# chongkuiqi/S2ANet

Measured on AMD Instinct MI355X. Metric: 1024x1024 DOTA chips/sec (R-50-FPN S2ANet inference), higher is better.
Workload: dtype f16; 1 GPU; BASELINE configs[2]: full R-50-FPN S2ANet inference, batch 8 of 1024x1024 synthetic uint8 chips per GPU; 3 independent batches in flight on 3 HIP streams; global_batch=8, num_classes=15, weights=seeded random init of the reference architecture; odm_cls bias calibrated, nms_candidate_cap=160000, nms_candidates_dropped=0, distinct_input_batches=3, fam_cls_branch=True, hip_graph=False, batches_in_flight=3, parallelism=dp1 (one process per GPU)

## Files before the change

include/s2anet_hip.h:

```cpp
#ifndef S2ANET_HIP_H_
#define S2ANET_HIP_H_

#include <stddef.h>
#include <stdint.h>

#ifdef __cplusplus
extern "C" {
#endif

#define S2A_OK 0
#define S2A_EINVAL (-1)
#define S2A_EWORKSPACE (-2)
#define S2A_EHIP (-3)
#define S2A_ENOTIMPL (-4)

#define S2A_DTYPE_F32 0
#define S2A_DTYPE_F16 1
#define S2A_DTYPE_F64 2

#define S2A_LAYOUT_NCHW 0
#define S2A_LAYOUT_NHWC 1

typedef void* s2a_stream_t;

// ... 237 lines not shown
                                                int64_t out_channels);
int s2a_deform_conv_backward(int dtype, const void* input, const void* offset, const void* grad_output, const void* weight,
                             float* grad_input_f32, void* grad_offset, float* grad_weight_f32, float scale, int64_t batch,
                             int64_t channels, int64_t height, int64_t width, int64_t out_channels, void* workspace,
                             size_t workspace_bytes, s2a_stream_t stream);
int s2a_deform_conv_backward_typed(int dtype, const void* input, const void* offset, const void* grad_output,
                                   const void* weight, void* grad_input, void* grad_offset, float* grad_weight_f32,
                                   float scale, int64_t batch, int64_t channels, int64_t height, int64_t width,
                                   int64_t out_channels, void* workspace, size_t workspace_bytes, s2a_stream_t stream);

int s2a_conv3x3_tail1x1_f16(const void* x, const void* weight_frag, const void* bias, const void* tail_weight_frag,
                            const void* tail_bias, const void* residual, void* out, const void* chain_weight_frag,
                            const void* chain_bias, void* chain_out, int64_t chain_channels, int64_t batch, int64_t channels,
                            int64_t mid_channels, int64_t out_channels, int64_t height, int64_t width,
                            s2a_stream_t stream);

int s2a_conv1x1_chain_f16(const void* x, const void* weight_frag, const void* bias, const void* residual, void* out,
                          const void* chain_weight_frag, const void* chain_bias, void* chain_out, int64_t chain_channels,
                          int64_t batch, int64_t channels, int64_t out_channels, int64_t height, int64_t width,
                          s2a_stream_t stream);

int s2a_conv1x1_add_up2_f16(const void* x, const void* weight_frag, const void* bias, const void* coarse,
                            void* out, int64_t batch, int64_t channels, int64_t height, int64_t width,
                            int64_t out_channels, s2a_stream_t stream);

int64_t s2a_pyramid_pixels(const s2a_pyramid* pyr, int64_t batch);
int s2a_conv3x3_pyramid_f16(const void* x, const void* weight_frag, const void* bias, const void* residual,
                            void* out, int64_t batch, int64_t channels, int64_t out_channels, int relu,
                            const s2a_pyramid* pyr, s2a_stream_t stream);
int s2a_conv3x3_head_pyramid_f16(const void* x, const void* weight_frag, const void* bias, void* out,
// ... 115 lines not shown
```

s2anet_amd/_lib.py:

```python
import ctypes
import os
import subprocess

import torch

_HERE = os.path.dirname(os.path.abspath(__file__))
LIB_PATH = os.environ.get("S2A_LIB_PATH") or os.path.join(_HERE, "libs2anet_hip.so")

OK, EINVAL, EWORKSPACE, EHIP, ENOTIMPL = 0, -1, -2, -3, -4
DTYPE_F32, DTYPE_F16, DTYPE_F64 = 0, 1, 2
LAYOUT_NCHW, LAYOUT_NHWC = 0, 1

c_i64, c_int, c_f32, c_sz, c_vp = (ctypes.c_int64, ctypes.c_int, ctypes.c_float, ctypes.c_size_t,
                                   ctypes.c_void_p)


class DcnParams(ctypes.Structure):
    _fields_ = [("batch", c_i64), ("channels", c_i64), ("height", c_i64), ("width", c_i64),
                ("out_channels", c_i64),
                ("kW", c_int), ("kH", c_int), ("dW", c_int), ("dH", c_int), ("padW", c_int),
                ("padH", c_int), ("dilationW", c_int), ("dilationH", c_int), ("group", c_int),
                ("deformable_group", c_int), ("dtype", c_int), ("offset_dtype", c_int),
                ("layout", c_int), ("relu", c_int)]

# ... 129 lines not shown
    "s2a_deform_conv_backward_typed": (c_int, [c_int, c_vp, c_vp, c_vp, c_vp, c_vp, c_vp, c_vp, c_f32, c_i64, c_i64, c_i64, c_i64,
                                               c_i64, c_vp, c_sz, c_vp]),
    "s2a_deform_conv_backward_input_f32_workspace_bytes": (c_sz, [c_i64, c_i64, c_i64, c_i64, c_i64]),
    "s2a_deform_conv_backward_weight_f32_workspace_bytes": (c_sz, [c_i64, c_i64, c_i64, c_i64, c_i64]),
    "s2a_deform_conv_backward_weight_f32": (c_int, [c_vp, c_vp, c_vp, c_vp, c_f32, c_i64, c_i64, c_i64, c_i64, c_i64,
                                                    c_vp, c_sz, c_vp]),
    "s2a_deform_conv_backward_input_f32": (c_int, [c_vp, c_vp, c_vp, c_vp, c_vp, c_vp, c_i64, c_i64, c_i64, c_i64, c_i64,
                                                   c_vp, c_sz, c_vp]),
    "s2a_deform_conv_backward_weight_f16": (c_int, [c_vp, c_vp, c_vp, c_vp, c_i64, c_i64, c_i64, c_i64, c_i64, c_vp, c_sz, c_vp]),
    "s2a_deform_conv_backward_input_f16": (c_int, [c_vp, c_vp, c_vp, c_vp, c_vp, c_vp, c_i64, c_i64, c_i64, c_i64, c_i64,
                                           c_vp, c_sz, c_vp]),
    "s2a_deformable_im2col": (c_int, [c_vp, c_vp, c_vp, ctypes.POINTER(DcnParams), c_vp]),
    "s2a_deformable_col2im": (c_int, [c_vp, c_vp, c_vp, ctypes.POINTER(DcnParams), c_vp]),
    "s2a_deformable_col2im_coord": (c_int, [c_vp, c_vp, c_vp, c_vp, ctypes.POINTER(DcnParams), c_vp]),
    "s2a_conv3x3_tail1x1_f16": (c_int, [c_vp] * 10 + [c_i64] * 7 + [c_vp]),
    "s2a_conv1x1_chain_f16": (c_int, [c_vp] * 8 + [c_i64] * 6 + [c_vp]),
    "s2a_conv1x1_add_up2_f16": (c_int, [c_vp, c_vp, c_vp, c_vp, c_vp, c_i64, c_i64, c_i64, c_i64, c_i64, c_vp]),
    "s2a_pyramid_pixels": (c_i64, [ctypes.POINTER(Pyramid), c_i64]),
    "s2a_conv3x3_pyramid_f16": (c_int, [c_vp, c_vp, c_vp, c_vp, c_vp, c_i64, c_i64, c_i64, c_int,
                                        ctypes.POINTER(Pyramid), c_vp]),
    "s2a_conv3x3_head_pyramid_f16": (c_int, [c_vp, c_vp, c_vp, c_vp, c_vp, c_vp, c_vp, c_i64, c_i64, c_i64, c_int,
                                             ctypes.POINTER(Pyramid), c_vp]),
    "s2a_conv3x3_narrow_pyramid_f16": (c_int, [c_vp, c_vp, c_vp, c_vp, c_i64, c_i64, c_i64, c_int, ctypes.POINTER(Pyramid), c_vp]),
    "s2a_orconv_pool_pyramid_f16": (c_int, [c_vp, c_vp, c_vp, c_vp, c_vp, c_i64, c_i64, c_i64, ctypes.POINTER(Pyramid), c_vp]),
    "s2a_conv_wino_packed_elems": (c_i64, [c_i64, c_i64]),
    "s2a_conv_wino_pack_weight_f16": (c_int, [c_vp, c_i64, c_i64, c_vp, c_vp]),
    "s2a_conv3x3_wino_pyramid_f16": (c_int, [c_vp, c_vp, c_vp, c_vp, c_vp, c_i64, c_i64, c_i64, c_int,
                                             ctypes.POINTER(Pyramid), c_vp]),
    "s2a_quantize_e4m3": (c_int, [c_vp, c_vp, c_i64, c_i64, c_f32, c_vp]),
    "s2a_conv_pack_weight_fp8": (c_int, [c_vp, c_i64, c_i64, c_vp, c_vp]),
# ... 102 lines not shown
```

s2anet_amd/csrc/conv_ops.hip:

```cpp
#include <hip/hip_fp16.h>
#include <hip/hip_runtime.h>

#include <algorithm>
#include <cstdlib>
#include <type_traits>

#include "common.hpp"
#include "mfma_common.hpp"

namespace s2a {
namespace {

__global__ void k_pack_weight_frag(const _Float16* __restrict__ w, int O, int C, _Float16* __restrict__ wp,
                                   int taps = 9) {
  int64_t e = (int64_t)blockIdx.x * blockDim.x + threadIdx.x;
  int64_t total = (int64_t)O * C * taps;
  if (e >= total) return;
  const int G = O / 64;
  int j = (int)(e & 7);
  int lane = (int)((e >> 3) & 63);
  int kk = (int)((e >> 9) & 3);
  int mt = (int)((e >> 11) & 1);
  int64_t r = e >> 12;
  int g = (int)(r % G);
// ... 8 lines not shown

struct ConvExtra {
  _Float16* pool_out;
  const _Float16* head_w;
  const _Float16* head_b;
  _Float16* head_out;
  int store_main;
  const _Float16* tail_w;
  const _Float16* tail_b;
  const _Float16* tail_res;
  _Float16* tail_out;
  const _Float16* chain_w;
  const _Float16* chain_b;
  _Float16* chain_out;
  int chain_O;
};

template <int TAPS, int OG, int PH = 1, int SD = 1, bool TAIL = false, int HT = 0>
struct ConvCfg {
  static constexpr int kTH = (SD == 2 || HT) ? 4 : 8 * PH;
  static constexpr int kPos = (SD == 2 || HT) ? 64 : 128 * PH;
  static constexpr int kWaves = 4 * PH;
  static constexpr int kPW = SD == 2 ? 33 : kCPW;
  static constexpr int kNT = (kPos / 32) * OG / 4 / PH;
  static constexpr int kPix = TAPS == 9 ? ((kTH - 1) * SD + 3) * kPW : kPos;
  static constexpr int kDma = (kPix * 9 + 63) / 64;
  static constexpr int kPatchBytes = kDma * 1024;
  static constexpr int kOutRowB = OG * 128 + 16;
  static constexpr bool kWLds = PH == 2 && TAPS == 9;
  static constexpr int kWBuf = OG * 8192;
  static constexpr int kLoop0 = 2 * kPatchBytes + (kWLds ? 2 * kWBuf : 0);
  static constexpr int kLoop = (kWLds && OG == 1 && kPatchBytes + 9 * 8192 > kLoop0) ? kPatchBytes + 9 * 8192 : kLoop0;
  static constexpr int kLds0 = (kLoop > kPos * kOutRowB) ? kLoop : kPos * kOutRowB;
  static constexpr int kTailRowB = 528;
  static constexpr int kLds = (TAIL && kPos * kTailRowB > kLds0) ? kPos * kTailRowB : kLds0;
  static constexpr int kBiasBytes = TAIL ? 1024 : 512;
  static constexpr int kJ = (kDma + kWaves - 1) / kWaves;
};

template <int TAPS, int OG, int PH = 1, int SD = 1, bool TAIL = false, int HT = 0>
__global__ __launch_bounds__(256 * PH, PH == 1 ? 2 : 1) void k_conv_f16(const _Float16* __restrict__ x_,
                                                     const _Float16* __restrict__ wfrag,
                                                     const _Float16* __restrict__ bias,
                                                     const _Float16* __restrict__ residual_,
                                                     _Float16* __restrict__ out_, int64_t Ntot_, int C,
                                                     int H_, int W_, int Ho_, int Wo_, int cstride, int O,
                                                     int relu, unsigned x_bytes_, LevelTab lt, int res_up,
                                                     ConvExtra ex) {
  _Float16* pool_out_ = ex.pool_out;
  using T = _Float16;
  using V = f16x8;
  using Cfg = ConvCfg<TAPS, OG, PH, SD, TAIL, HT>;
  constexpr int NT = Cfg::kNT;
  static_assert(NT >= 1, "unsupported tile / group combination");
  static_assert(!HT || (TAPS == 9 && PH == 1 && SD == 1 && !TAIL), "half tiles: plain 3x3 / stride 1");
  static_assert(!TAIL || (TAPS == 9 && OG == 1 && SD == 1), "the fused 1x1 tail follows a 64-map 3x3/s1");
  constexpr int WPG = 4 / OG;
  constexpr int kThreads_ = 256 * PH;
  extern __shared__ __attribute__((aligned(16))) char smem[];
  const int tid = threadIdx.x, lane = tid & 63, wave = tid >> 6;
  const int wave4 = wave & 3, blk = wave >> 2;
  int64_t tile = xcd_remap(blockIdx.x, gridDim.x);
  const T* x = x_;
  const T* residual = residual_;
  T* out = out_;
  int64_t Ntot = Ntot_;
  int H = H_, W = W_, Ho = Ho_, Wo = Wo_;
  unsigned x_bytes = x_bytes_;
  if (TAPS == 9 && lt.n > 1) {
    int t0 = 0, p0 = 0;
#pragma unroll
// ... 136 lines not shown
      return;
    }
#pragma unroll
    for (int kk = 0; kk < 4; kk++) {
      V pf[NT];
#pragma unroll
      for (int b = 0; b < NT; b++) pf[b] = *reinterpret_cast<const V*>(P + fbase[b] + toff + kk * 32);
#pragma unroll
      for (int a = 0; a < 2; a++)
#pragma unroll
        for (int b = 0; b < NT; b++)
          acc[a][b] = __builtin_amdgcn_mfma_f32_32x32x16_f16(wv[a][kk], pf[b], acc[a][b], 0, 0, 0);
    }
  };

  constexpr bool kEarlyRes = TAIL && Cfg::kWLds;
  constexpr int NI2 = TAIL ? Cfg::kPos * 32 / kThreads_ : 1;
  unsigned off2[NI2];
  V r2[NI2];
  auto tail_res_issue = [&]() {
    const __amdgpu_buffer_rsrc_t rr = __builtin_amdgcn_make_buffer_rsrc(
        const_cast<T*>(ex.tail_res ? ex.tail_res : ex.tail_out), 0, (int)((uint64_t)Ntot * 256 * 2), 0x00020000);
#pragma unroll
    for (int i = 0; i < NI2; i++) {
      const int idx = tid + kThreads_ * i, pos = idx >> 5, col = idx & 31;
      const int64_t gp = tile_pos(tile, pos, Cfg::kTH, Ho, Wo, HWo, Ntot);
      off2[i] = gp >= 0 ? (unsigned)((gp * 256 + col * 8) * 2) : 0x80000000u;
      r2[i] = __builtin_bit_cast(V, __builtin_amdgcn_raw_buffer_load_b128(rr, (int)(ex.tail_res ? off2[i] : 0x80000000u), 0, 0));
    }
  };
  const int nstage = TAPS * CC, last = nstage - 1;
  if constexpr (Cfg::kWLds) {
    char* wb = smem + 2 * Cfg::kPatchBytes;
    const __amdgpu_buffer_rsrc_t rw = __builtin_amdgcn_make_buffer_rsrc(
// ... 154 lines not shown
          const int och = grp * 64 + 32 * a + 8 * rq + 4 * (lane >> 5);
          const h4e bq = *reinterpret_cast<const h4e*>(s_bias + och);
#pragma unroll
          for (int b = 0; b < NT; b++) {
            int pos = 128 * blk + 32 * (sub * NT + b) + lp;
            *reinterpret_cast<h4e*>(s_out + pos * Cfg::kOutRowB + och * 2) =
                quad(acc[a][b][rq * 4], acc[a][b][rq * 4 + 1], acc[a][b][rq * 4 + 2], acc[a][b][rq * 4 + 3], bq);
          }
        }
    }
  };
  if (wave_active) {
    if (relu && !residual) stage_tile(std::true_type{}); else stage_tile(std::false_type{});
  }
  __syncthreads();
  if constexpr (TAIL) {
    f32x4 acc3s[4][8];
    {
#pragma unroll
      for (int a = 0; a < 4; a++)
#pragma unroll
        for (int b = 0; b < 8; b++)
#pragma unroll
          for (int r = 0; r < 4; r++) acc3s[a][b][r] = 0.f;
      const char* brow = s_out + (128 * blk + pix16) * Cfg::kOutRowB + (kg16 & 1) * 64 + (kg16 >> 1) * 16;
#pragma unroll
      for (int ks = 0; ks < 2; ks++)
#pragma unroll
        for (int bh = 0; bh < 8; bh += 4) {
          V pf[4];
#pragma unroll
          for (int b = 0; b < 4; b++) pf[b] = *reinterpret_cast<const V*>(brow + (bh + b) * 16 * Cfg::kOutRowB + ks * 32);
#pragma unroll
          for (int a = 0; a < 4; a++)
#pragma unroll
            for (int b = 0; b < 4; b++)
              acc3s[a][bh + b] = __builtin_amdgcn_mfma_f32_16x16x32_f16(wt[(a * 2 + ks) >> 2][(a * 2 + ks) & 3], pf[b], acc3s[a][bh + b], 0, 0, 0);
        }
    }
    if constexpr (!kEarlyRes) {
      const __amdgpu_buffer_rsrc_t rr = __builtin_amdgcn_make_buffer_rsrc(
          const_cast<T*>(ex.tail_res ? ex.tail_res : ex.tail_out), 0, (int)((uint64_t)Ntot * 256 * 2), 0x00020000);
#pragma unroll
      for (int i = 0; i < NI2; i++) {
        const int idx = tid + kThreads_ * i, pos = idx >> 5, col = idx & 31;
        const int64_t gp = tile_pos(tile, pos, Cfg::kTH, Ho, Wo, HWo, Ntot);
        off2[i] = gp >= 0 ? (unsigned)((gp * 256 + col * 8) * 2) : 0x80000000u;
        r2[i] = __builtin_bit_cast(V, __builtin_amdgcn_raw_buffer_load_b128(rr, (int)(ex.tail_res ? off2[i] : 0x80000000u), 0, 0));
      }
    }
    __syncthreads();
    {
      using h4 = __attribute__((ext_vector_type(4))) _Float16;
#pragma unroll
      for (int a = 0; a < 4; a++) {
        const int och = wave4 * 64 + 16 * a + 4 * kg16;
        const h4 bq = *reinterpret_cast<const h4*>(s_bias + 64 + och);
#pragma unroll
        for (int b = 0; b < 8; b++) {
          h4 v4;
#pragma unroll
          for (int e = 0; e < 4; e++) v4[e] = (_Float16)(acc3s[a][b][e] + (float)bq[e]);
          *reinterpret_cast<h4*>(s_out + (128 * blk + 16 * b + pix16) * Cfg::kTailRowB + och * 2) = v4;
        }
      }
    }
    __syncthreads();
    const int O3 = ex.chain_O, MT = max(O3 / 32, 1);
    const int nper = (Cfg::kPos / 32) * MT / Cfg::kWaves;
    const int mt = wave % MT, nt0 = (wave / MT) * nper;
    const int G3 = O3 / 64;
    V aw[16];
    if (ex.chain_w) {
      const V* cwp = reinterpret_cast<const V*>(ex.chain_w) + lane + ((mt >> 1) * 8 + (mt & 1) * 4) * 64;
#pragma unroll
      for (int c4 = 0; c4 < 4; c4++)
#pragma unroll
        for (int kk = 0; kk < 4; kk++) aw[c4 * 4 + kk] = cwp[(c4 * G3 * 8 + kk) * 64];
    }
#pragma unroll
    for (int i = 0; i < NI2; i++) {
      const int idx = tid + kThreads_ * i, pos = idx >> 5, col = idx & 31;
      V v = *reinterpret_cast<const V*>(s_out + pos * Cfg::kTailRowB + col * 16);
#pragma unroll
      for (int e = 0; e < 8; e += 2) {
        h2e p2 = {(_Float16)((float)v[e] + (float)r2[i][e]), (_Float16)((float)v[e + 1] + (float)r2[i][e + 1])};
        p2 = __builtin_elementwise_max(p2, h2e{(_Float16)0.f, (_Float16)0.f});
        v[e] = p2[0];
        v[e + 1] = p2[1];
      }
      if (off2[i] != 0x80000000u) *reinterpret_cast<V*>(reinterpret_cast<char*>(ex.tail_out) + off2[i]) = v;
      if (ex.chain_w) *reinterpret_cast<V*>(s_out + pos * Cfg::kTailRowB + col * 16) = v;
    }
    if (ex.chain_w) {
      f32x16 c2[4];
#pragma unroll
      for (int j = 0; j < 4; j++)
#pragma unroll
        for (int r = 0; r < 16; r++) c2[j][r] = 0.f;
      __syncthreads();
#pragma unroll
      for (int c4 = 0; c4 < 4; c4++)
#pragma unroll
        for (int kk = 0; kk < 4; kk++)
#pragma unroll
          for (int j = 0; j < 4; j++)
            if (j < nper) {
              const V bf = *reinterpret_cast<const V*>(s_out + (32 * (nt0 + j) + (lane & 31)) * Cfg::kTailRowB +
                                                       (c4 * 64 + kk * 16 + (lane >> 5) * 8) * 2);
              c2[j] = __builtin_amdgcn_mfma_f32_32x32x16_f16(aw[c4 * 4 + kk], bf, c2[j], 0, 0, 0);
            }
      __syncthreads();
      const int rowb = O3 * 2 + 16;
#pragma unroll
      for (int j = 0; j < 4; j++)
// ... 521 lines not shown
#pragma unroll
      for (int e = 0; e < 8; e++) v[e] = (_Float16)0.f;
      if (col < 2) v = *reinterpret_cast<const V*>(so + pos * 32 + col * 16);
      if (y < cur.H && xq < cur.W) *reinterpret_cast<V*>(out + (cur.base + (int64_t)y * cur.W + xq) * 64 + col * 8) = v;
    }
  }
}

}
}

using namespace s2a;

namespace s2a {
namespace {
template <int TAPS, int OG, int PH = 1, int SD = 1, bool TAIL = false, int HT = 0>
int launch_conv(const _Float16* x, const _Float16* wfrag, const _Float16* bias, const _Float16* residual,
                _Float16* out, int64_t B, int C, int H, int W, int Ho, int Wo, int cstride, int O, int relu,
                hipStream_t st, const LevelTab* levels = nullptr, int64_t level_tiles = 0, int res_up = 0,
                ConvExtra ex = ConvExtra{nullptr, nullptr, nullptr, nullptr, 1}) {
  using Cfg = ConvCfg<TAPS, OG, PH, SD, TAIL, HT>;
  const int64_t Ntot = B * (int64_t)Ho * Wo;
  int64_t tiles = TAPS == 9 ? B * ((Wo + 15) / 16) * ((Ho + Cfg::kTH - 1) / Cfg::kTH) : (Ntot + Cfg::kPos - 1) / Cfg::kPos;
  LevelTab lt = {};
  if (levels) { lt = *levels; tiles = level_tiles; }
  dim3 grid((unsigned)tiles, (unsigned)((O + 64 * OG - 1) / (64 * OG)));
  auto kern = k_conv_f16<TAPS, OG, PH, SD, TAIL, HT>;
  S2A_HIP(hipFuncSetAttribute(reinterpret_cast<const void*>(kern), hipFuncAttributeMaxDynamicSharedMemorySize, Cfg::kLds + Cfg::kBiasBytes));
  kern<<<grid, 256 * PH, Cfg::kLds + Cfg::kBiasBytes, st>>>(x, wfrag, bias, residual, out, Ntot, C, H, W, Ho, Wo, cstride, O, relu,
                                     (unsigned)((uint64_t)B * H * W * C * 2), lt, res_up, ex);
  S2A_LAUNCH_CHECK();
  return S2A_OK;
}

struct ConvCall {
  const _Float16 *x, *wfrag, *bias, *residual;
  _Float16* out;
  int64_t B;
  int C, H, W, Ho, Wo, cstride, O, relu;
  hipStream_t st;
  const LevelTab* levels = nullptr;
  int64_t level_tiles = 0;
  int res_up = 0;
  ConvExtra ex = ConvExtra{nullptr, nullptr, nullptr, nullptr, 1};
  template <int TAPS, int OG, int PH = 1, int SD = 1, bool TAIL = false, int HT = 0>
  int run() const {
    return launch_conv<TAPS, OG, PH, SD, TAIL, HT>(x, wfrag, bias, residual, out, B, C, H, W, Ho, Wo, cstride, O, relu, st, levels,
                                                   level_tiles, res_up, ex);
  }
};
}
}

extern "C" int s2a_conv_nhwc_f16(const void* x, const void* weight_frag, const void* bias, const void* residual,
                                 void* out, int64_t batch, int64_t channels, int64_t height, int64_t width,
                                 int64_t out_channels, int ksize, int stride, int relu, s2a_stream_t stream) {
  S2A_CHECK_ARG(batch >= 0 && channels > 0 && out_channels > 0 && height > 0 && width > 0, "conv: bad shape");
  S2A_CHECK_ARG(ksize == 3 || ksize == 1, "conv: kernel size must be 1 or 3");
  S2A_CHECK_ARG(stride == 1 || stride == 2, "conv: stride must be 1 or 2");
  S2A_CHECK_ARG(!(ksize == 3 && stride == 2) || out_channels % 128 == 0, "conv: 3x3 stride 2 needs out_channels % 128 == 0");
  S2A_CHECK_ARG((channels % 64 == 0 || channels == 32) && out_channels % 64 == 0,
                "conv: channels must be 32 or a multiple of 64, out_channels a multiple of 64");
// ... 76 lines not shown
    S2A_CHECK_ARG(((uintptr_t)chain_weight_frag % 16) == 0 && ((uintptr_t)chain_bias % 8) == 0 && ((uintptr_t)chain_out % 16) == 0,
                  "conv3x3_tail1x1: chain tensors must be 16-byte aligned");
    ex.chain_w = (const _Float16*)chain_weight_frag;
    ex.chain_b = (const _Float16*)chain_bias;
    ex.chain_out = (_Float16*)chain_out;
    ex.chain_O = (int)chain_channels;
  }
  int ph = batch * ((width + 15) / 16) * ((height + 15) / 16) >= 256 ? 2 : 1;
  if (const char* f = getenv("S2A_CONV_PH_NARROW")) ph = atoi(f) == 2 ? 2 : 1;
  const ConvCall c{(const _Float16*)x, (const _Float16*)weight_frag, (const _Float16*)bias, nullptr, (_Float16*)out, batch, 64,
                   (int)height, (int)width, (int)height, (int)width, 1, 64, 1, as_stream(stream), nullptr, 0, 0, ex};
  if (ph == 2) return c.run<9, 1, 2, 1, true>();
  return c.run<9, 1, 1, 1, true>();
}

namespace s2a {
namespace {
template <int CC, int O3>
int launch_conv1x1_chain(const _Float16* x, const _Float16* wfrag, const _Float16* bias, const _Float16* residual, _Float16* out,
                         const _Float16* cw, const _Float16* cb, _Float16* cout, int64_t P, hipStream_t st) {
  constexpr int K = 64 * CC;
  const int loop = CC * 64 * kRowBytes + 64 * 528 + 512;
  const int tail = 64 * (O3 * 2 + 16);
  const int lds = loop > tail ? loop : tail;
  auto kern = k_conv1x1_chain_f16<CC, O3>;
  S2A_HIP(hipFuncSetAttribute(reinterpret_cast<const void*>(kern), hipFuncAttributeMaxDynamicSharedMemorySize, lds));
  kern<<<dim3((unsigned)((P + 63) / 64)), 256, lds, st>>>(x, wfrag, bias, residual, out, cw, cb, cout, P,
                                                          (unsigned)((uint64_t)P * K * 2));
  S2A_LAUNCH_CHECK();
  return S2A_OK;
// ... 163 lines not shown
```

s2anet_amd/detector.py:

```python
import math
import os

import torch
import torch.nn as nn
import torch.nn.functional as F

from .fused import Conv3Chain, FusedConv2d, bottleneck_chain_ok, bottleneck_tail, bottleneck_tail_ok, conv3_chain_ok
from .head import S2ANetHead


class BottleNeck(nn.Module):
    expansion = 4

    def __init__(self, inplanes, planes, stride=1, downsample=None):
        super().__init__()
        self.conv1 = nn.Conv2d(inplanes, planes, kernel_size=1, stride=1, bias=False)
        self.bn1 = nn.BatchNorm2d(planes)
        self.conv2 = nn.Conv2d(planes, planes, kernel_size=3, stride=stride, padding=1, bias=False)
        self.bn2 = nn.BatchNorm2d(planes)
        self.conv3 = nn.Conv2d(planes, planes * self.expansion, kernel_size=1, bias=False)
        self.bn3 = nn.BatchNorm2d(planes * self.expansion)
        self.relu = nn.ReLU(inplace=True)
        self.downsample = downsample
        self.stride = stride

    def forward(self, x):
        return self.forward_chain(x)[0]

    def forward_chain(self, x, pre=None, nxt=None):
        residual = x
        if isinstance(self.conv3, FusedConv2d):
            out = pre if pre is not None else self.conv1(x)
            if self.downsample is not None:
                residual = self.downsample(x)
            if bottleneck_tail_ok(out, self.conv2, self.conv3, residual):
                if isinstance(nxt, BottleNeck) and bottleneck_chain_ok(nxt.conv1):
                    return bottleneck_tail(out, self.conv2, self.conv3, residual, nxt.conv1)
                return bottleneck_tail(out, self.conv2, self.conv3, residual), None
            if isinstance(nxt, BottleNeck) and conv3_chain_ok(self.conv3, nxt.conv1):
                ch = Conv3Chain(nxt.conv1)
                return self.conv3(self.conv2(out), residual, chain=ch), ch.out
            return self.conv3(self.conv2(out), residual), None
        return self._forward_plain(x), None

    def _forward_plain(self, x):
        residual = x
        out = self.relu(self.bn1(self.conv1(x)))
# ... 270 lines not shown
```

s2anet_amd/fused.py:

```python
import torch
import torch.nn as nn
import torch.nn.functional as F

from . import _lib


def _needs_grad(*tensors):
    return torch.is_grad_enabled() and any(t is not None and t.requires_grad for t in tensors)


def bias_act_(y, bias, residual=None, relu=False, out=None):
    _lib.require_cuda(y, bias, residual)
    B, C, H, W = y.shape
    if out is not None:
        assert out.shape == y.shape and out.dtype == y.dtype and out.permute(0, 2, 3, 1).is_contiguous()
    grad = _needs_grad(y, bias, residual)
    if grad and out is not None:
        raise RuntimeError("bias_act_(out=...) writes a caller's buffer and has no backward: call it under torch.no_grad()")
    ok = (not grad and y.is_contiguous(memory_format=torch.channels_last) and
          C % (8 if y.dtype == torch.float16 else 4) == 0 and y.dtype in (torch.float16, torch.float32) and
          (residual is None or (residual.shape == y.shape and residual.dtype == y.dtype and
                                residual.is_contiguous(memory_format=torch.channels_last))))
    if not ok:
        y = y + bias.view(1, -1, 1, 1).to(y.dtype)
# ... 72 lines not shown
    return out


def conv_wino_f16(x, packed_wino, bias, out_channels, relu=False, pool=False):
    from .pyramid import PyramidLayout, conv3x3_wino
    B, C, H, W = x.shape
    assert x.dtype == torch.float16 and x.is_contiguous(memory_format=torch.channels_last)
    lay = PyramidLayout(B, [(H, W)], [1.0])
    b = None if bias is None else bias.to(torch.float16).contiguous()
    r = conv3x3_wino(lay, x.permute(0, 2, 3, 1).reshape(-1, C), packed_wino, b, out_channels, relu, pool)
    if pool:
        return (r[0].view(B, H, W, out_channels).permute(0, 3, 1, 2), r[1].view(B, H, W, out_channels // 8).permute(0, 3, 1, 2))
    return r.view(B, H, W, out_channels).permute(0, 3, 1, 2)


def conv_f16(x, packed_weight, bias, out_channels, ksize, stride=1, relu=False, residual=None, out=None, chain=None):
    B, C, H, W = x.shape
    Ho, Wo = (H - 1) // stride + 1, (W - 1) // stride + 1
    O_real = out_channels
    if out_channels < 64:
        assert residual is None
        out_channels = 64
    if out is None:
        out = torch.empty((B, out_channels, Ho, Wo), dtype=torch.float16, device=x.device,
                          memory_format=torch.channels_last)
    else:
        assert out.shape == (B, out_channels, Ho, Wo) and out.dtype == torch.float16 and \
            out.permute(0, 2, 3, 1).is_contiguous()
    b = None if bias is None else bias.to(torch.float16).contiguous()
    if b is not None and b.numel() < out_channels:
        b = torch.cat([b, b.new_zeros(out_channels - b.numel())])
    if residual is not None:
        assert residual.shape == out.shape and residual.dtype == torch.float16 and \
            residual.is_contiguous(memory_format=torch.channels_last)
    if chain is not None and ksize == 1 and stride == 1 and relu and b is not None and \
            (C, out_channels, chain.conv.out_channels) in CONV3_CHAIN_SHAPES and out.numel() * 2 < (1 << 31):
        wc, bc, _ = chain.conv.packed_args()
        chain.out = torch.empty((B, chain.conv.out_channels, H, W), dtype=torch.float16, device=x.device,
                                memory_format=torch.channels_last)
        with torch.cuda.device(x.device):
            _lib.check(_lib.lib().s2a_conv1x1_chain_f16(_lib.ptr(x), _lib.ptr(packed_weight), _lib.ptr(b), _lib.ptr(residual),
                                                        _lib.ptr(out), _lib.ptr(wc), _lib.ptr(bc), _lib.ptr(chain.out),
                                                        chain.conv.out_channels, B, C, out_channels, H, W,
                                                        _lib.stream_ptr(x.device)))
        return out
    with torch.cuda.device(x.device):
        _lib.check(_lib.lib().s2a_conv_nhwc_f16(_lib.ptr(x), _lib.ptr(packed_weight), _lib.ptr(b), _lib.ptr(residual),
                                                _lib.ptr(out), B, C, H, W, out_channels, int(ksize), int(stride),
                                                int(bool(relu)), _lib.stream_ptr(x.device)))
    return out if O_real == out_channels else out[:, :O_real]


CONV3_CHAIN_SHAPES = {(128, 512, 128), (128, 512, 256), (256, 1024, 256)}


class Conv3Chain:

    def __init__(self, conv):
        self.conv, self.out = conv, None


def conv3_chain_ok(conv3, conv1):
    import os
    def plain(c):
        return (isinstance(c, FusedConv2d) and tuple(c.kernel_size) == (1, 1) and tuple(c.stride) == (1, 1) and
                tuple(c.padding) == (0, 0) and tuple(c.dilation) == (1, 1) and c.groups == 1 and c.bias is not None and
                c.fuse_relu and c.weight.dtype == torch.float16)
    return (not torch.is_grad_enabled() and not os.environ.get("S2A_NO_CONV3_CHAIN") and plain(conv3) and plain(conv1) and
            conv1.in_channels == conv3.out_channels and
            (conv3.in_channels, conv3.out_channels, conv1.out_channels) in CONV3_CHAIN_SHAPES)


def bottleneck_tail_ok(x, conv2, conv3, residual):
    import os
    return (not torch.is_grad_enabled() and not os.environ.get("S2A_NO_FUSED_TAIL") and
            isinstance(conv2, FusedConv2d) and isinstance(conv3, FusedConv2d) and
            conv2.in_channels == 64 and conv2.out_channels == 64 and conv3.out_channels == 256 and
            conv2.fuse_relu and conv3.fuse_relu and conv2.bias is not None and conv3.bias is not None and
            own_conv_ok(x, 64, 64, conv2.kernel_size, conv2.stride, conv2.padding, conv2.dilation, conv2.groups) and
            tuple(conv2.kernel_size) == (3, 3) and tuple(conv2.stride) == (1, 1) and
            tuple(conv3.kernel_size) == (1, 1) and tuple(conv3.stride) == (1, 1) and
            x.shape[0] * x.shape[2] * x.shape[3] * 512 < (1 << 31) and
            (residual is None or (residual.dtype == torch.float16 and residual.shape[1] == 256 and
                                  residual.shape[2:] == x.shape[2:] and
                                  residual.is_contiguous(memory_format=torch.channels_last))))


def bottleneck_chain_ok(conv1):
    import os
    return (isinstance(conv1, FusedConv2d) and not os.environ.get("S2A_NO_TAIL_CHAIN") and
            conv1.in_channels == 256 and conv1.out_channels in (64, 128) and tuple(conv1.kernel_size) == (1, 1) and
            tuple(conv1.stride) == (1, 1) and tuple(conv1.padding) == (0, 0) and conv1.groups == 1 and
            conv1.fuse_relu and conv1.bias is not None and conv1.weight.dtype == torch.float16)


def bottleneck_tail(x, conv2, conv3, residual=None, chain=None):
    B, C, H, W = x.shape
    out = torch.empty((B, 256, H, W), dtype=torch.float16, device=x.device, memory_format=torch.channels_last)
    w2, b2, _ = conv2.packed_args()
    w3, b3, _ = conv3.packed_args()
# ... 189 lines not shown
        if not hasattr(self, "_packed"):
            self._packed = PackedWeightCache()
        w, sc = self._packed.get_fp8(self.weight, in_scale)
        return w, sc, self._packed.get_bias_f32(self.bias), self.out_channels

    def wino_ok(self):
        return (tuple(self.kernel_size) == (3, 3) and tuple(self.stride) == (1, 1) and tuple(self.padding) == (1, 1) and
                tuple(self.dilation) == (1, 1) and self.groups == 1 and self.out_channels % 64 == 0 and
                self.in_channels % 32 == 0)

    def packed_args_wino(self):
        if not hasattr(self, "_packed"):
            self._packed = PackedWeightCache()
        return self._packed.get_wino(self.weight), self._packed.get_bias(self.bias, self.out_channels), self.out_channels

    def forward(self, x, residual=None, out=None, chain=None):
        if out is None and self.own_grad and _needs_grad(x, self.weight, self.bias, residual) and \
                train_conv_ok(x, self, residual):
            return FusedConvFunction.apply(x, self.weight, self.bias, residual, self.fuse_relu)
        if out is not None:
            assert x.is_cuda and self.bias is not None and not torch.is_grad_enabled() and not own_conv_ok(
                x, self.in_channels, self.out_channels, self.kernel_size, self.stride, self.padding, self.dilation, self.groups)
            y = F.conv2d(x, self.weight, None, self.stride, self.padding, self.dilation, self.groups)
            return bias_act_(y, self.bias, residual, self.fuse_relu, out=out)
        if not torch.is_grad_enabled() and own_conv_ok(
                x, self.in_channels, self.out_channels, self.kernel_size, self.stride, self.padding,
                self.dilation, self.groups) and (residual is None or (
                    residual.dtype == torch.float16 and residual.is_contiguous(memory_format=torch.channels_last))):
            if not hasattr(self, "_packed"):
                self._packed = PackedWeightCache()
            kw = {} if chain is None else {"chain": chain}
            return conv_f16(x, self._packed.get(self.weight), self._packed.get_bias(self.bias, max(64, self.out_channels)),
                            self.out_channels, self.kernel_size[0], self.stride[0], self.fuse_relu, residual, **kw)
        if (not x.is_cuda) or self.bias is None:
            y = super().forward(x)
            if residual is not None:
                y = y + residual
            return F.relu(y) if self.fuse_relu else y
        y = F.conv2d(x, self.weight, None, self.stride, self.padding, self.dilation, self.groups)
        return bias_act_(y, self.bias, residual, self.fuse_relu)


def stem_pack_weight(weight):
    w = weight.detach().to(torch.float16).contiguous()
    assert tuple(w.shape) == (64, 3, 7, 7)
    L = _lib.lib()
# ... 19 lines not shown
```

Baseline: 1983 chips/s.

## Fuse downsample 1x1 conv into bottleneck 3x3+1x1 tail kernel

Adds a DS variant of the fused 3x3 -> 1x1 bottleneck tail kernel. It also computes the 64->256 downsampling 1x1 on the block input inside the same kernel, adds it as the residual, applies ReLU and optionally chains into the next block's conv1. This removes a separate downsample conv launch and the write and read of its 256-channel residual tensor. It only applies to the stride-1 64-channel first block of layer1. The kernel now also writes the mid activation and carries extra register and MFMA work.

```diff
diff --git a/include/s2anet_hip.h b/include/s2anet_hip.h
--- a/include/s2anet_hip.h
+++ b/include/s2anet_hip.h
@@ -275,6 +275,13 @@
                             const void* chain_bias, void* chain_out, int64_t chain_channels, int64_t batch, int64_t channels,
                             int64_t mid_channels, int64_t out_channels, int64_t height, int64_t width,
                             s2a_stream_t stream);
+
+int s2a_conv3x3_tail1x1_ds_f16(const void* x, const void* weight_frag, const void* bias, void* mid_out,
+                               const void* tail_weight_frag, const void* tail_bias, const void* ds_x,
+                               const void* ds_weight_frag, const void* ds_bias, void* out, const void* chain_weight_frag,
+                               const void* chain_bias, void* chain_out, int64_t chain_channels, int64_t batch,
+                               int64_t channels, int64_t mid_channels, int64_t out_channels, int64_t height, int64_t width,
+                               s2a_stream_t stream);
 
 int s2a_conv1x1_chain_f16(const void* x, const void* weight_frag, const void* bias, const void* residual, void* out,
                           const void* chain_weight_frag, const void* chain_bias, void* chain_out, int64_t chain_channels,
diff --git a/s2anet_amd/_lib.py b/s2anet_amd/_lib.py
--- a/s2anet_amd/_lib.py
+++ b/s2anet_amd/_lib.py
@@ -167,6 +167,7 @@
     "s2a_deformable_col2im": (c_int, [c_vp, c_vp, c_vp, ctypes.POINTER(DcnParams), c_vp]),
     "s2a_deformable_col2im_coord": (c_int, [c_vp, c_vp, c_vp, c_vp, ctypes.POINTER(DcnParams), c_vp]),
     "s2a_conv3x3_tail1x1_f16": (c_int, [c_vp] * 10 + [c_i64] * 7 + [c_vp]),
+    "s2a_conv3x3_tail1x1_ds_f16": (c_int, [c_vp] * 13 + [c_i64] * 7 + [c_vp]),
     "s2a_conv1x1_chain_f16": (c_int, [c_vp] * 8 + [c_i64] * 6 + [c_vp]),
     "s2a_conv1x1_add_up2_f16": (c_int, [c_vp, c_vp, c_vp, c_vp, c_vp, c_i64, c_i64, c_i64, c_i64, c_i64, c_vp]),
     "s2a_pyramid_pixels": (c_i64, [ctypes.POINTER(Pyramid), c_i64]),
diff --git a/s2anet_amd/csrc/conv_ops.hip b/s2anet_amd/csrc/conv_ops.hip
--- a/s2anet_amd/csrc/conv_ops.hip
+++ b/s2anet_amd/csrc/conv_ops.hip
@@ -46,6 +46,10 @@
   const _Float16* chain_b;
   _Float16* chain_out;
   int chain_O;
+  const _Float16* ds_x;
+  const _Float16* ds_w;
+  const _Float16* ds_b;
+  _Float16* mid_out;
 };
 
 template <int TAPS, int OG, int PH = 1, int SD = 1, bool TAIL = false, int HT = 0>
@@ -70,7 +74,7 @@
   static constexpr int kJ = (kDma + kWaves - 1) / kWaves;
 };
 
-template <int TAPS, int OG, int PH = 1, int SD = 1, bool TAIL = false, int HT = 0>
+template <int TAPS, int OG, int PH = 1, int SD = 1, bool TAIL = false, int HT = 0, bool DS = false>
 __global__ __launch_bounds__(256 * PH, PH == 1 ? 2 : 1) void k_conv_f16(const _Float16* __restrict__ x_,
                                                      const _Float16* __restrict__ wfrag,
                                                      const _Float16* __restrict__ bias,
@@ -87,6 +91,7 @@
   static_assert(NT >= 1, "unsupported tile / group combination");
   static_assert(!HT || (TAPS == 9 && PH == 1 && SD == 1 && !TAIL), "half tiles: plain 3x3 / stride 1");
   static_assert(!TAIL || (TAPS == 9 && OG == 1 && SD == 1), "the fused 1x1 tail follows a 64-map 3x3/s1");
+  static_assert(!DS || TAIL, "the in-place down-sampling 1x1 belongs to the fused tail");
   constexpr int WPG = 4 / OG;
   constexpr int kThreads_ = 256 * PH;
   extern __shared__ __attribute__((aligned(16))) char smem[];
@@ -253,10 +258,22 @@
     }
   };
 
-  constexpr bool kEarlyRes = TAIL && Cfg::kWLds;
+  constexpr bool kEarlyRes = TAIL && Cfg::kWLds && !DS;
   constexpr int NI2 = TAIL ? Cfg::kPos * 32 / kThreads_ : 1;
   unsigned off2[NI2];
   V r2[NI2];
+  auto ds_frag_issue = [&]() {
+    const __amdgpu_buffer_rsrc_t rd = __builtin_amdgcn_make_buffer_rsrc(
+        const_cast<T*>(ex.ds_x), 0, (int)((uint64_t)Ntot * 64 * 2), 0x00020000);
+#pragma unroll
+    for (int b = 0; b < 8; b++) {
+      const int64_t gp = tile_pos(tile, 128 * blk + 16 * b + pix16, Cfg::kTH, Ho, Wo, HWo, Ntot);
+      const unsigned o = gp >= 0 ? (unsigned)(gp * 128 + (kg16 & 1) * 64 + (kg16 >> 1) * 16) : 0x80000000u;
+#pragma unroll
+      for (int ks = 0; ks < 2; ks++)
+        r2[b * 2 + ks] = __builtin_bit_cast(V, __builtin_amdgcn_raw_buffer_load_b128(rd, (int)(o + ks * 32), 0, 0));
+    }
+  };
   auto tail_res_issue = [&]() {
     const __amdgpu_buffer_rsrc_t rr = __builtin_amdgcn_make_buffer_rsrc(
         const_cast<T*>(ex.tail_res ? ex.tail_res : ex.tail_out), 0, (int)((uint64_t)Ntot * 256 * 2), 0x00020000);
@@ -441,6 +458,15 @@
     if (relu && !residual) stage_tile(std::true_type{}); else stage_tile(std::false_type{});
   }
   __syncthreads();
+  if constexpr (DS) {
+#pragma unroll
+    for (int i = 0; i < Cfg::kPos * 8 / kThreads_; i++) {
+      const int idx = tid + kThreads_ * i, pos = idx >> 3, col = idx & 7;
+      const int64_t gp = tile_pos(tile, pos, Cfg::kTH, Ho, Wo, HWo, Ntot);
+      if (gp >= 0)
+        *reinterpret_cast<V*>(ex.mid_out + gp * 64 + col * 8) = *reinterpret_cast<const V*>(s_out + pos * Cfg::kOutRowB + col * 16);
+    }
+  }
   if constexpr (TAIL) {
     f32x4 acc3s[4][8];
     {
@@ -465,7 +491,8 @@
               acc3s[a][bh + b] = __builtin_amdgcn_mfma_f32_16x16x32_f16(wt[(a * 2 + ks) >> 2][(a * 2 + ks) & 3], pf[b], acc3s[a][bh + b], 0, 0, 0);
         }
     }
-    if constexpr (!kEarlyRes) {
+    if constexpr (DS) ds_frag_issue();
+    if constexpr (!kEarlyRes && !DS) {
       const __amdgpu_buffer_rsrc_t rr = __builtin_amdgcn_make_buffer_rsrc(
           const_cast<T*>(ex.tail_res ? ex.tail_res : ex.tail_out), 0, (int)((uint64_t)Ntot * 256 * 2), 0x00020000);
 #pragma unroll
@@ -476,6 +503,14 @@
         r2[i] = __builtin_bit_cast(V, __builtin_amdgcn_raw_buffer_load_b128(rr, (int)(ex.tail_res ? off2[i] : 0x80000000u), 0, 0));
       }
     }
+    h4e dsb[4];
+    if constexpr (DS) {
+      const V* tp = reinterpret_cast<const V*>(ex.ds_w) + (int64_t)wave4 * 8 * 64 + ((lane >> 4) & 1) * 128 + (lane >> 5) * 32 + (lane & 15);
+#pragma unroll
+      for (int f = 0; f < 8; f++) wt[f >> 2][f & 3] = tp[((f >> 2) * 4 + (f & 1)) * 64 + ((f >> 1) & 1) * 16];
+#pragma unroll
+      for (int a = 0; a < 4; a++) dsb[a] = *reinterpret_cast<const h4e*>(ex.ds_b + wave4 * 64 + 16 * a + 4 * kg16);
+    }
     __syncthreads();
     {
       using h4 = __attribute__((ext_vector_type(4))) _Float16;
@@ -489,6 +524,39 @@
 #pragma unroll
           for (int e = 0; e < 4; e++) v4[e] = (_Float16)(acc3s[a][b][e] + (float)bq[e]);
           *reinterpret_cast<h4*>(s_out + (128 * blk + 16 * b + pix16) * Cfg::kTailRowB + och * 2) = v4;
+        }
+      }
+    }
+    if constexpr (DS) {
+      __builtin_amdgcn_sched_barrier(0);
+#pragma unroll
+      for (int a = 0; a < 4; a++)
+#pragma unroll
+        for (int b = 0; b < 8; b++)
+#pragma unroll
+          for (int r = 0; r < 4; r++) acc3s[a][b][r] = 0.f;
+#pragma unroll
+      for (int ks = 0; ks < 2; ks++)
+#pragma unroll
+        for (int a = 0; a < 4; a++)
+#pragma unroll
+          for (int b = 0; b < 8; b++)
+            acc3s[a][b] = __builtin_amdgcn_mfma_f32_16x16x32_f16(wt[(a * 2 + ks) >> 2][(a * 2 + ks) & 3], r2[b * 2 + ks], acc3s[a][b], 0, 0, 0);
+#pragma unroll
+      for (int a = 0; a < 4; a++) {
+        const int och = wave4 * 64 + 16 * a + 4 * kg16;
+#pragma unroll
+        for (int b = 0; b < 8; b++) {
+          char* q = s_out + (128 * blk + 16 * b + pix16) * Cfg::kTailRowB + och * 2;
+          const h4e v = *reinterpret_cast<const h4e*>(q);
+          h4e rd;
+#pragma unroll
+          for (int e = 0; e < 4; e++) rd[e] = (_Float16)(acc3s[a][b][e] + (float)dsb[a][e]);
+          h2e lo = {(_Float16)((float)v[0] + (float)rd[0]), (_Float16)((float)v[1] + (float)rd[1])};
+          h2e hi = {(_Float16)((float)v[2] + (float)rd[2]), (_Float16)((float)v[3] + (float)rd[3])};
+          lo = __builtin_elementwise_max(lo, h2e{(_Float16)0.f, (_Float16)0.f});
+          hi = __builtin_elementwise_max(hi, h2e{(_Float16)0.f, (_Float16)0.f});
+          *reinterpret_cast<h4e*>(q) = h4e{lo[0], lo[1], hi[0], hi[1]};
         }
       }
     }
@@ -505,19 +573,29 @@
 #pragma unroll
         for (int kk = 0; kk < 4; kk++) aw[c4 * 4 + kk] = cwp[(c4 * G3 * 8 + kk) * 64];
     }
-#pragma unroll
-    for (int i = 0; i < NI2; i++) {
-      const int idx = tid + kThreads_ * i, pos = idx >> 5, col = idx & 31;
-      V v = *reinterpret_cast<const V*>(s_out + pos * Cfg::kTailRowB + col * 16);
-#pragma unroll
-      for (int e = 0; e < 8; e += 2) {
-        h2e p2 = {(_Float16)((float)v[e] + (float)r2[i][e]), (_Float16)((float)v[e + 1] + (float)r2[i][e + 1])};
-        p2 = __builtin_elementwise_max(p2, h2e{(_Float16)0.f, (_Float16)0.f});
-        v[e] = p2[0];
-        v[e + 1] = p2[1];
-      }
-      if (off2[i] != 0x80000000u) *reinterpret_cast<V*>(reinterpret_cast<char*>(ex.tail_out) + off2[i]) = v;
-      if (ex.chain_w) *reinterpret_cast<V*>(s_out + pos * Cfg::kTailRowB + col * 16) = v;
+    if constexpr (DS) {
+#pragma unroll
+      for (int i = 0; i < NI2; i++) {
+        const int idx = tid + kThreads_ * i, pos = idx >> 5, col = idx & 31;
+        const int64_t gp = tile_pos(tile, pos, Cfg::kTH, Ho, Wo, HWo, Ntot);
+        if (gp >= 0)
+          *reinterpret_cast<V*>(ex.tail_out + gp * 256 + col * 8) = *reinterpret_cast<const V*>(s_out + pos * Cfg::kTailRowB + col * 16);
+      }
+    } else {
+#pragma unroll
+      for (int i = 0; i < NI2; i++) {
+        const int idx = tid + kThreads_ * i, pos = idx >> 5, col = idx & 31;
+        V v = *reinterpret_cast<const V*>(s_out + pos * Cfg::kTailRowB + col * 16);
+#pragma unroll
+        for (int e = 0; e < 8; e += 2) {
+          h2e p2 = {(_Float16)((float)v[e] + (float)r2[i][e]), (_Float16)((float)v[e + 1] + (float)r2[i][e + 1])};
+          p2 = __builtin_elementwise_max(p2, h2e{(_Float16)0.f, (_Float16)0.f});
+          v[e] = p2[0];
+          v[e + 1] = p2[1];
+        }
+        if (off2[i] != 0x80000000u) *reinterpret_cast<V*>(reinterpret_cast<char*>(ex.tail_out) + off2[i]) = v;
+        if (ex.chain_w) *reinterpret_cast<V*>(s_out + pos * Cfg::kTailRowB + col * 16) = v;
+      }
     }
     if (ex.chain_w) {
       f32x16 c2[4];
@@ -525,7 +603,7 @@
       for (int j = 0; j < 4; j++)
 #pragma unroll
         for (int r = 0; r < 16; r++) c2[j][r] = 0.f;
-      __syncthreads();
+      if constexpr (!DS) __syncthreads();
 #pragma unroll
       for (int c4 = 0; c4 < 4; c4++)
 #pragma unroll
@@ -1077,7 +1155,7 @@
 
 namespace s2a {
 namespace {
-template <int TAPS, int OG, int PH = 1, int SD = 1, bool TAIL = false, int HT = 0>
+template <int TAPS, int OG, int PH = 1, int SD = 1, bool TAIL = false, int HT = 0, bool DS = false>
 int launch_conv(const _Float16* x, const _Float16* wfrag, const _Float16* bias, const _Float16* residual,
                 _Float16* out, int64_t B, int C, int H, int W, int Ho, int Wo, int cstride, int O, int relu,
                 hipStream_t st, const LevelTab* levels = nullptr, int64_t level_tiles = 0, int res_up = 0,
@@ -1088,7 +1166,7 @@
   LevelTab lt = {};
   if (levels) { lt = *levels; tiles = level_tiles; }
   dim3 grid((unsigned)tiles, (unsigned)((O + 64 * OG - 1) / (64 * OG)));
-  auto kern = k_conv_f16<TAPS, OG, PH, SD, TAIL, HT>;
+  auto kern = k_conv_f16<TAPS, OG, PH, SD, TAIL, HT, DS>;
   S2A_HIP(hipFuncSetAttribute(reinterpret_cast<const void*>(kern), hipFuncAttributeMaxDynamicSharedMemorySize, Cfg::kLds + Cfg::kBiasBytes));
   kern<<<grid, 256 * PH, Cfg::kLds + Cfg::kBiasBytes, st>>>(x, wfrag, bias, residual, out, Ntot, C, H, W, Ho, Wo, cstride, O, relu,
                                      (unsigned)((uint64_t)B * H * W * C * 2), lt, res_up, ex);
@@ -1106,9 +1184,9 @@
   int64_t level_tiles = 0;
   int res_up = 0;
   ConvExtra ex = ConvExtra{nullptr, nullptr, nullptr, nullptr, 1};
-  template <int TAPS, int OG, int PH = 1, int SD = 1, bool TAIL = false, int HT = 0>
+  template <int TAPS, int OG, int PH = 1, int SD = 1, bool TAIL = false, int HT = 0, bool DS = false>
   int run() const {
-    return launch_conv<TAPS, OG, PH, SD, TAIL, HT>(x, wfrag, bias, residual, out, B, C, H, W, Ho, Wo, cstride, O, relu, st, levels,
+    return launch_conv<TAPS, OG, PH, SD, TAIL, HT, DS>(x, wfrag, bias, residual, out, B, C, H, W, Ho, Wo, cstride, O, relu, st, levels,
                                                    level_tiles, res_up, ex);
   }
 };
@@ -1215,6 +1293,51 @@
   return c.run<9, 1, 1, 1, true>();
 }
 
+extern "C" int s2a_conv3x3_tail1x1_ds_f16(const void* x, const void* weight_frag, const void* bias, void* mid_out,
+                                          const void* tail_weight_frag, const void* tail_bias, const void* ds_x,
+                                          const void* ds_weight_frag, const void* ds_bias, void* out,
+                                          const void* chain_weight_frag, const void* chain_bias, void* chain_out,
+                                          int64_t chain_channels, int64_t batch, int64_t channels, int64_t mid_channels,
+                                          int64_t out_channels, int64_t height, int64_t width, s2a_stream_t stream) {
+  S2A_CHECK_ARG(batch >= 0 && height > 0 && width > 0, "conv3x3_tail1x1_ds: bad shape");
+  S2A_CHECK_ARG(channels == 64 && mid_channels == 64 && out_channels == 256,
+                "conv3x3_tail1x1_ds: built for the 64 -> 64 -> 256 bottleneck tail with a 64 -> 256 down-sampling 1x1");
+  S2A_CHECK_ARG((uint64_t)batch * height * width * out_channels * 2 < (1ull << 31) && height < 32000 && width < 32000,
+                "conv3x3_tail1x1_ds: tensor too large for 32-bit offsets");
+  if (batch == 0) return S2A_OK;
+  S2A_CHECK_ARG(x && weight_frag && bias && mid_out && tail_weight_frag && tail_bias && ds_x && ds_weight_frag && ds_bias && out,
+                "conv3x3_tail1x1_ds: NULL tensor");
+  S2A_CHECK_ARG(((uintptr_t)x % 16) == 0 && ((uintptr_t)out % 16) == 0 && ((uintptr_t)weight_frag % 16) == 0 &&
+                ((uintptr_t)tail_weight_frag % 16) == 0 && ((uintptr_t)bias % 8) == 0 && ((uintptr_t)tail_bias % 8) == 0 &&
+                ((uintptr_t)mid_out % 16) == 0 && ((uintptr_t)ds_x % 16) == 0 && ((uintptr_t)ds_weight_frag % 16) == 0 &&
+                ((uintptr_t)ds_bias % 8) == 0, "conv3x3_tail1x1_ds: tensors must be 16-byte aligned");
+  ConvExtra ex{};
+  ex.store_main = 0;
+  ex.tail_w = (const _Float16*)tail_weight_frag;
+  ex.tail_b = (const _Float16*)tail_bias;
+  ex.tail_out = (_Float16*)out;
+  ex.ds_x = (const _Float16*)ds_x;
+  ex.ds_w = (const _Float16*)ds_weight_frag;
+  ex.ds_b = (const _Float16*)ds_bias;
+  ex.mid_out = (_Float16*)mid_out;
+  if (chain_weight_frag || chain_bias || chain_out) {
+    S2A_CHECK_ARG(chain_weight_frag && chain_bias && chain_out, "conv3x3_tail1x1_ds: chain filter, bias and output go together");
+    S2A_CHECK_ARG(chain_channels == 64 || chain_channels == 128, "conv3x3_tail1x1_ds: the chained 1x1 has 64 or 128 maps");
+    S2A_CHECK_ARG(((uintptr_t)chain_weight_frag % 16) == 0 && ((uintptr_t)chain_bias % 8) == 0 && ((uintptr_t)chain_out % 16) == 0,
+                  "conv3x3_tail1x1_ds: chain tensors must be 16-byte aligned");
+    ex.chain_w = (const _Float16*)chain_weight_frag;
+    ex.chain_b = (const _Float16*)chain_bias;
+    ex.chain_out = (_Float16*)chain_out;
+    ex.chain_O = (int)chain_channels;
+  }
+  int ph = batch * ((width + 15) / 16) * ((height + 15) / 16) >= 256 ? 2 : 1;
+  if (const char* f = getenv("S2A_CONV_PH_NARROW")) ph = atoi(f) == 2 ? 2 : 1;
+  const ConvCall c{(const _Float16*)x, (const _Float16*)weight_frag, (const _Float16*)bias, nullptr, (_Float16*)out, batch, 64,
+                   (int)height, (int)width, (int)height, (int)width, 1, 64, 1, as_stream(stream), nullptr, 0, 0, ex};
+  if (ph == 2) return c.run<9, 1, 2, 1, true, 0, true>();
+  return c.run<9, 1, 1, 1, true, 0, true>();
+}
+
 namespace s2a {
 namespace {
 template <int CC, int O3>
diff --git a/s2anet_amd/detector.py b/s2anet_amd/detector.py
--- a/s2anet_amd/detector.py
+++ b/s2anet_amd/detector.py
@@ -5,7 +5,8 @@
 import torch.nn as nn
 import torch.nn.functional as F
 
-from .fused import Conv3Chain, FusedConv2d, bottleneck_chain_ok, bottleneck_tail, bottleneck_tail_ok, conv3_chain_ok
+from .fused import (Conv3Chain, FusedConv2d, TailDownsample, bottleneck_chain_ok, bottleneck_tail, bottleneck_tail_ok,
+                    conv3_chain_ok, tail_downsample_ok)
 from .head import S2ANetHead
 
 
@@ -31,6 +32,14 @@
         residual = x
         if isinstance(self.conv3, FusedConv2d):
             out = pre if pre is not None else self.conv1(x)
+            if self.downsample is not None and tail_downsample_ok(out, x, self.conv2, self.conv3, self.downsample):
+                chained = isinstance(nxt, BottleNeck) and bottleneck_chain_ok(nxt.conv1)
+                ds = self.downsample[0] if isinstance(self.downsample, nn.Sequential) else self.downsample
+                t = TailDownsample(self.conv3, ds, x, nxt.conv1 if chained else None)
+                mid = self.conv2(out, tail=t)
+                if t.out is not None:
+                    return t.out, t.next
+                return self.conv3(mid, self.downsample(x)), None
             if self.downsample is not None:
                 residual = self.downsample(x)
             if bottleneck_tail_ok(out, self.conv2, self.conv3, residual):
diff --git a/s2anet_amd/fused.py b/s2anet_amd/fused.py
--- a/s2anet_amd/fused.py
+++ b/s2anet_amd/fused.py
@@ -110,7 +110,8 @@
     return r.view(B, H, W, out_channels).permute(0, 3, 1, 2)
 
 
-def conv_f16(x, packed_weight, bias, out_channels, ksize, stride=1, relu=False, residual=None, out=None, chain=None):
+def conv_f16(x, packed_weight, bias, out_channels, ksize, stride=1, relu=False, residual=None, out=None, chain=None,
+             tail=None):
     B, C, H, W = x.shape
     Ho, Wo = (H - 1) // stride + 1, (W - 1) // stride + 1
     O_real = out_channels
@@ -140,6 +141,24 @@
                                                         chain.conv.out_channels, B, C, out_channels, H, W,
                                                         _lib.stream_ptr(x.device)))
         return out
+    if tail is not None and ksize == 3 and stride == 1 and relu and b is not None and residual is None and \
+            C == 64 and out_channels == 64 and O_real == 64 and tail.x.shape == (B, 64, H, W) and \
+            B * H * W * 512 < (1 << 31):
+        w3, b3, _ = tail.conv3.packed_args()
+        wd, bd, _ = tail.downsample.packed_args()
+        wc = bc = None
+        if tail.chain is not None:
+            wc, bc, _ = tail.chain.packed_args()
+            tail.next = torch.empty((B, tail.chain.out_channels, H, W), dtype=torch.float16, device=x.device,
+                                    memory_format=torch.channels_last)
+        tail.out = torch.empty((B, 256, H, W), dtype=torch.float16, device=x.device, memory_format=torch.channels_last)
+        with torch.cuda.device(x.device):
+            _lib.check(_lib.lib().s2a_conv3x3_tail1x1_ds_f16(
+                _lib.ptr(x), _lib.ptr(packed_weight), _lib.ptr(b), _lib.ptr(out), _lib.ptr(w3), _lib.ptr(b3),
+                _lib.ptr(tail.x), _lib.ptr(wd), _lib.ptr(bd), _lib.ptr(tail.out), _lib.ptr(wc), _lib.ptr(bc),
+                _lib.ptr(tail.next), 0 if tail.chain is None else tail.chain.out_channels, B, 64, 64, 256, H, W,
+                _lib.stream_ptr(x.device)))
+        return out
     with torch.cuda.device(x.device):
         _lib.check(_lib.lib().s2a_conv_nhwc_f16(_lib.ptr(x), _lib.ptr(packed_weight), _lib.ptr(b), _lib.ptr(residual),
                                                 _lib.ptr(out), B, C, H, W, out_channels, int(ksize), int(stride),
@@ -154,6 +173,13 @@
 
     def __init__(self, conv):
         self.conv, self.out = conv, None
+
+
+class TailDownsample:
+
+    def __init__(self, conv3, downsample, x, chain=None):
+        self.conv3, self.downsample, self.x, self.chain = conv3, downsample, x, chain
+        self.out = self.next = None
 
 
 def conv3_chain_ok(conv3, conv1):
@@ -180,6 +206,19 @@
             (residual is None or (residual.dtype == torch.float16 and residual.shape[1] == 256 and
                                   residual.shape[2:] == x.shape[2:] and
                                   residual.is_contiguous(memory_format=torch.channels_last))))
+
+
+def tail_downsample_ok(x1, x, conv2, conv3, downsample):
+    import os
+    ds = downsample[0] if isinstance(downsample, torch.nn.Sequential) and len(downsample) == 1 else downsample
+    return (not torch.is_grad_enabled() and not os.environ.get("S2A_NO_TAIL_DS") and
+            bottleneck_tail_ok(x1, conv2, conv3, None) and isinstance(ds, FusedConv2d) and
+            tuple(ds.kernel_size) == (1, 1) and tuple(ds.stride) == (1, 1) and tuple(ds.padding) == (0, 0) and
+            tuple(ds.dilation) == (1, 1) and ds.groups == 1 and ds.in_channels == 64 and ds.out_channels == 256 and
+            ds.bias is not None and not ds.fuse_relu and ds.weight.dtype == torch.float16 and
+            x.is_cuda and x.dtype == torch.float16 and x.dim() == 4 and x.shape[1] == 64 and
+            x.shape[0] == x1.shape[0] and x.shape[2:] == x1.shape[2:] and
+            x.is_contiguous(memory_format=torch.channels_last))
 
 
 def bottleneck_chain_ok(conv1):
@@ -399,7 +438,7 @@
             self._packed = PackedWeightCache()
         return self._packed.get_wino(self.weight), self._packed.get_bias(self.bias, self.out_channels), self.out_channels
 
-    def forward(self, x, residual=None, out=None, chain=None):
+    def forward(self, x, residual=None, out=None, chain=None, tail=None):
         if out is None and self.own_grad and _needs_grad(x, self.weight, self.bias, residual) and \
                 train_conv_ok(x, self, residual):
             return FusedConvFunction.apply(x, self.weight, self.bias, residual, self.fuse_relu)
@@ -415,6 +454,8 @@
             if not hasattr(self, "_packed"):
                 self._packed = PackedWeightCache()
             kw = {} if chain is None else {"chain": chain}
+            if tail is not None:
+                kw["tail"] = tail
             return conv_f16(x, self._packed.get(self.weight), self._packed.get_bias(self.bias, max(64, self.out_channels)),
                             self.out_channels, self.kernel_size[0], self.stride[0], self.fuse_relu, residual, **kw)
         if (not x.is_cuda) or self.bias is None:
```

After: 1973 chips/s. No clear change (-0.5%).
